# Napoliee/Expressive-FastSpeech2-Mandarin

Measured on AMD Instinct MI355X. Metric: mel-frames/sec/GPU (batch-64 synth) at 1/2/4/8 MI355X; RTF, higher is better.
Workload: dtype bf16; 1 GPU; cfg2: batch=64 x 64 phonemes per GPU, ESD-Chinese-Singing-MFA model.yaml, FastSpeech2.forward eval bf16; global_batch=64, seq_len=64, mel_frames_per_gpu_batch=24883, T_max=430, parallelism=dp1 (independent shards, no collective), hip_graph=True

## Files before the change

expressive-fastspeech2-mandarin_amd/csrc/ffn.hip:

```cpp
#include <cstdlib>
#include <type_traits>
#include <utility>

#include "conv_common.h"
#include "fs2_common.h"

namespace {

#ifndef FFN_TRACE
#define FFN_TRACE 0
#endif
#ifndef FFN_ABLATE
#define FFN_ABLATE 0
#endif

constexpr int kD = 256;
constexpr int kChunk = 256;
constexpr int kUnit = 4096;
constexpr int kDepth = 4;

struct FfnArgs {
  ConvArgs e;
  const bf16 *w;
  const float *b1;
// ... 946 lines not shown
      if (hf == 0) {
#pragma unroll
        for (int i = 0; i < N; ++i) xp[i * 64] = pv[i];
      }
      __builtin_amdgcn_s_waitcnt(kLgkm0);
      __builtin_amdgcn_sched_barrier(0);
      __builtin_amdgcn_s_barrier();
      __builtin_amdgcn_sched_barrier(0);
      if (hf == 1) {
#pragma unroll
        for (int i = 0; i < N; ++i) pv[i] = (xp[i * 64] + sv[0][i]) + sv[1][i];
      }
    }
  };
  const rsrc_t wr = make_rsrc(p.w, p.w_bytes);
  auto tile_dma_range = [&](const void *src, uint32_t bytes, int64_t stride, int off, int i0, int i1) {
    const rsrc_t sr = make_rsrc(src, bytes);
    const uint32_t srow = (uint32_t)stride * 2u;
#pragma unroll
    for (int i = i0; i < i1; ++i) {
      const int pc = wv + NW * i;
      const int o = pc * 1024 + lane * 16;
      const int r = o / XPITCH, within = o - r * XPITCH;
      const int gm = m0 - pad + r;
      const bool ok = r < XROWS && within < 512 && gm >= 0 && gm < M;
      __builtin_amdgcn_raw_ptr_buffer_load_lds(
          sr, (__attribute__((address_space(3))) void *)(smem + off + pc * 1024), 16,
          ok ? (uint32_t)gm * srow + (uint32_t)within : kOOB, 0, 0, 0);
    }
  };
  constexpr uint32_t W2_BASE = (uint32_t)(F * KS * kD * 2);
  const uint32_t lane_off = (uint32_t)lane * 16u + (uint32_t)hf * 2048u;
  auto base1 = [&](int c) { return (uint32_t)((c * 4 + w) * NK1) * (uint32_t)kUnit; };
  auto base2 = [&](int c) { return W2_BASE + (uint32_t)(w * (F / 32) + c * NK2) * (uint32_t)kUnit; };
  bf16x8 pa[DEPTH][JB];
  auto load_at = [&](auto S, uint32_t so) {
    constexpr int s = decltype(S)::value;
    if (FFN_ABLATE & 2) return;
    __builtin_amdgcn_sched_barrier(0);
#pragma unroll
    for (int jb = 0; jb < JB; ++jb) {
      auto v = __builtin_amdgcn_raw_buffer_load_b128(wr, lane_off + jb * 1024, (FFN_ABLATE & 8) ? 0u : so, 0);
      pa[s][jb] = __builtin_bit_cast(bf16x8, v);
    }
    __builtin_amdgcn_sched_barrier(0);
  };
  auto ring_start = [&]() {
    static_for<DEPTH>([&](auto I) { load_at(I, base1(c0) + (uint32_t)(decltype(I)::value * kUnit)); });
  };
  {
    const int hr = lane & 15, hq = lane >> 4;
    if (wv < 3) vec_dma(wv == 0 ? p.bfc : wv == 1 ? p.g1 : p.be1, 0, smem + VEC0_OFF + wv * 1024);
    const rsrc_t fr = make_rsrc(p.wfc, (uint32_t)(kD * kD * 2));
    const uint32_t lane_o = lane_off;
    bf16x8 wf[8][JB];
#pragma unroll
    for (int ks = 0; ks < 8; ++ks)
#pragma unroll
      for (int jb = 0; jb < JB; ++jb)
        wf[ks][jb] = __builtin_bit_cast(bf16x8, __builtin_amdgcn_raw_buffer_load_b128(
                                                    fr, lane_o + (uint32_t)(jb * 1024), (uint32_t)((w * 8 + ks) * kUnit), 0));
    constexpr int PRE_SPLIT = (64 * XPITCH + 1023) / 1024 / NW + 1;
    static_assert(NW * PRE_SPLIT * 1024 >= 64 * XPITCH && PRE_SPLIT <= XP_PER_WAVE, "row pass 0 pieces");
    tile_dma_range(p.att, p.att_bytes, p.as, ATT_OFF, 0, PRE_SPLIT);
    tile_dma_range(a.x, a.x_bytes, a.xs, X_OFF, 0, PRE_SPLIT);
    tile_dma_range(p.att, p.att_bytes, p.as, ATT_OFF, PRE_SPLIT, XP_PER_WAVE);
    tile_dma_range(a.x, a.x_bytes, a.xs, X_OFF, PRE_SPLIT, XP_PER_WAVE);
    stamp(21);
    __builtin_amdgcn_s_waitcnt(vm_imm(2 * (XP_PER_WAVE - PRE_SPLIT)));
    __builtin_amdgcn_s_waitcnt(kLgkm0);
    __builtin_amdgcn_s_barrier();
    stamp(22);
    float *red0 = reinterpret_cast<float *>(smem + RED0_OFF);
    static_for<(XROWS + 63) / 64>([&](auto PS) {
      constexpr int ps = decltype(PS)::value;
      if constexpr (ps == 1) {
        asm volatile("s_waitcnt vmcnt(0)" ::: "memory");
        __builtin_amdgcn_s_barrier();
      }
      f32x4 a0[JB][4];
#pragma unroll
      for (int jb = 0; jb < JB; ++jb)
#pragma unroll
        for (int mb = 0; mb < 4; ++mb) a0[jb][mb] = f32x4{0.f, 0.f, 0.f, 0.f};
#pragma unroll
      for (int ks = 0; ks < 8; ++ks) {
        bf16x8 fb[4];
#pragma unroll
        for (int mb = 0; mb < 4; ++mb) {
          const int r = min(64 * ps + 16 * mb + hr, XROWS - 1);
          fb[mb] = *reinterpret_cast<const bf16x8 *>(smem + ATT_OFF + r * XPITCH + ks * 64 + hq * 16);
        }
#pragma unroll
        for (int mb = 0; mb < 4; ++mb)
#pragma unroll
          for (int jb = 0; jb < JB; ++jb)
            a0[jb][mb] = __builtin_amdgcn_mfma_f32_16x16x32_bf16(wf[ks][jb], fb[mb], a0[jb][mb], 0, 0, 0);
      }
      float part[4] = {0.f, 0.f, 0.f, 0.f}, mean[4], var[4];
      float sv[JB][4];
#pragma unroll
      for (int jb = 0; jb < JB; ++jb) {
        const int n = col0 + jb * 16 + 4 * hq;
        const float4 bb = *reinterpret_cast<const float4 *>(smem + VEC0_OFF + 4 * n);
#pragma unroll
        for (int mb = 0; mb < 4; ++mb) {
          const int r = 64 * ps + 16 * mb + hr, gm = m0 - pad + r;
          const bool ok = r < XROWS && gm >= 0 && gm < M;
          bf16x4 xv = {(bf16)0.f, (bf16)0.f, (bf16)0.f, (bf16)0.f};
          if (ok) xv = *reinterpret_cast<const bf16x4 *>(smem + X_OFF + r * XPITCH + n * 2);
          f32x4 v = a0[jb][mb];
          v[0] = v[0] + bb.x + (float)xv[0];
          v[1] = v[1] + bb.y + (float)xv[1];
          v[2] = v[2] + bb.z + (float)xv[2];
          v[3] = v[3] + bb.w + (float)xv[3];
          a0[jb][mb] = v;
          if constexpr (NW == 8) {
            sv[jb][mb] = (v[0] + v[1]) + (v[2] + v[3]);
            part[mb] += sv[jb][mb];
          } else {
            part[mb] += (v[0] + v[1]) + (v[2] + v[3]);
          }
        }
      }
      auto reduce4 = [&](float (&pv)[4], float (&tot)[4]) {
        pair_sum(pv, sv);
        float t[4];
#pragma unroll
        for (int mb = 0; mb < 4; ++mb) t[mb] = __shfl_xor(pv[mb], 16, 64);
#pragma unroll
        for (int mb = 0; mb < 4; ++mb) pv[mb] += t[mb];
#pragma unroll
        for (int mb = 0; mb < 4; ++mb) t[mb] = __shfl_xor(pv[mb], 32, 64);
        if (NW == 4 || hf == 1) {
#pragma unroll
          for (int mb = 0; mb < 4; ++mb) red0[(mb * 16 + hr) * 4 + w] = pv[mb] + t[mb];
        }
        __builtin_amdgcn_s_waitcnt(kLgkm0);
        __builtin_amdgcn_s_barrier();
#pragma unroll
        for (int mb = 0; mb < 4; ++mb) {
          const float4 r4 = *reinterpret_cast<const float4 *>(red0 + (mb * 16 + hr) * 4);
          tot[mb] = (r4.x + r4.y) + (r4.z + r4.w);
        }
        __builtin_amdgcn_s_waitcnt(kLgkm0);
        __builtin_amdgcn_s_barrier();
      };
      reduce4(part, mean);
#pragma unroll
      for (int mb = 0; mb < 4; ++mb) {
        mean[mb] *= 1.0f / kD;
        float ss = 0.f;
#pragma unroll
        for (int jb = 0; jb < JB; ++jb) {
          f32x4 d = a0[jb][mb];
          d[0] -= mean[mb];
          d[1] -= mean[mb];
          d[2] -= mean[mb];
          d[3] -= mean[mb];
          a0[jb][mb] = d;
          if constexpr (NW == 8) {
            if constexpr (ps == 0)
              sv[jb][mb] = sumsq4<true>(d);
            else if (jb == 0 && mb < 3 && hf == 0)
              sv[jb][mb] = sumsq4<true>(d);
            else
              sv[jb][mb] = sumsq4<false>(d);
            ss += sv[jb][mb];
          } else {
            ss += (d[0] * d[0] + d[1] * d[1]) + (d[2] * d[2] + d[3] * d[3]);
          }
        }
        part[mb] = ss;
      }
      reduce4(part, var);
      float rstd[4], keep[4] = {1.f, 1.f, 1.f, 1.f};
#pragma unroll
      for (int mb = 0; mb < 4; ++mb) rstd[mb] = 1.0f / sqrtf(var[mb] * (1.0f / kD) + p.eps1);
      if (NW == 4 && a.lens != nullptr) {
#pragma unroll
        for (int mb = 0; mb < 4; ++mb) {
          const int gm = m0 - pad + 64 * ps + 16 * mb + hr;
          if (gm >= 0 && gm < M) {
            const int bb = gm / T;
            keep[mb] = (int64_t)(gm - bb * T) < a.lens[bb] ? 1.0f : 0.0f;
          }
        }
      }
#pragma unroll
      for (int jb = 0; jb < JB; ++jb) {
        const int n = col0 + jb * 16 + 4 * hq;
        const float4 g = *reinterpret_cast<const float4 *>(smem + VEC0_OFF + 4 * (kD + n));
        const float4 be = *reinterpret_cast<const float4 *>(smem + VEC0_OFF + 4 * (2 * kD + n));
#pragma unroll
        for (int mb = 0; mb < 4; ++mb) {
          const int r = 64 * ps + 16 * mb + hr;
          const f32x4 d = a0[jb][mb];
          bf16x4 o;
          o[0] = (bf16)((d[0] * rstd[mb] * g.x + be.x) * keep[mb]);
          o[1] = (bf16)((d[1] * rstd[mb] * g.y + be.y) * keep[mb]);
          o[2] = (bf16)((d[2] * rstd[mb] * g.z + be.z) * keep[mb]);
          o[3] = (bf16)((d[3] * rstd[mb] * g.w + be.w) * keep[mb]);
          if (r < XROWS) *reinterpret_cast<bf16x4 *>(smem + X_OFF + r * XPITCH + n * 2) = o;
        }
      }
      stamp(23 + ps);
    });
    __builtin_amdgcn_s_waitcnt(kLgkm0);
    __builtin_amdgcn_s_barrier();
    load_vectors();
    ring_start();
  }


  const int hrow0 = lane & 15;
  const int hi = lane >> 4;
  bf16x8 f0[MB], f1[MB];
  auto bases_x = [&](int tap, int (&ad)[MB]) {
    const int base = X_OFF + (hrow0 + tap) * XPITCH + hi * 16;
#pragma unroll
    for (int mb = 0; mb < MB; ++mb) {
      const int keep = (FFN_ABLATE & 16) ? -1 : __builtin_amdgcn_sbfe(vmask[mb], tap, 1);
      ad[mb] = (base + mb * 16 * XPITCH) & keep;
    }
  };
  auto issue_x = [&](const int (&ad)[MB], auto KSI, bf16x8 (&f)[MB]) {
    if (FFN_ABLATE & 4) return;
    constexpr int off = decltype(KSI)::value * 64;
#pragma unroll
    for (int mb = 0; mb < MB; ++mb) f[mb] = *reinterpret_cast<const bf16x8 *>(smem + ad[mb] + off);
  };
  auto read_h = [&](int q, bf16x8 (&f)[MB]) {
    if (FFN_ABLATE & 4) return;
    const char *hp = smem + H_OFF + hrow0 * 512 + (xchunk(hrow0, 4 * q + hi) << 4);
#pragma unroll
    for (int mb = 0; mb < MB; ++mb) f[mb] = *reinterpret_cast<const bf16x8 *>(hp + mb * 8192);
  };

  f32x4 acc1[JB][MB], acc2[JB][MB];
#pragma unroll
  for (int i = 0; i < JB; ++i)
#pragma unroll
    for (int j = 0; j < MB; ++j) {
      acc1[i][j] = f32x4{0.f, 0.f, 0.f, 0.f};
      acc2[i][j] = f32x4{0.f, 0.f, 0.f, 0.f};
    }
  auto mma = [&](f32x4 (&acc)[JB][MB], const bf16x8 (&fa)[JB], const bf16x8 (&fb)[MB]) {
    if (FFN_ABLATE & 1) return;
#pragma unroll
    for (int mb = 0; mb < MB; ++mb)
#pragma unroll
      for (int jb = 0; jb < JB; ++jb)
        acc[jb][mb] = __builtin_amdgcn_mfma_f32_16x16x32_bf16(fa[jb], fb[mb], acc[jb][mb], 0, 0, 0);
  };
  auto bar = []() {
    __builtin_amdgcn_sched_barrier(0);
    __builtin_amdgcn_s_barrier();
    __builtin_amdgcn_sched_barrier(0);
  };
  auto trace_dump = [&](int last) {
    if (FFN_TRACE) {
      uint64_t *o = S > 1 ? reinterpret_cast<uint64_t *>(static_cast<char *>(p.part) + p.part_bytes + 256u * blockIdx.x)
                          : reinterpret_cast<uint64_t *>(static_cast<char *>(a.out) + (size_t)(a.M - 1 - blockIdx.x) * a.os * 2);
      for (int i = 0; i < 25; ++i) o[i] = *reinterpret_cast<const uint64_t *>(smem + SMEM + 8 * i);
      o[28] = t_entry;
      o[29] = (uint64_t)split;
      o[30] = (uint64_t)last;
      o[31] = (uint64_t)25;
    }
  };
  stamp(0);

  auto write_h = [&](int c) {
    float z;
    asm volatile("v_mov_b32 %0, 0" : "=v"(z));
#pragma unroll
    for (int jb = 0; jb < JB; ++jb) {
      const int j = col0 + jb * 16 + 4 * hi;
      const float4 bb = *reinterpret_cast<const float4 *>(smem + B1_OFF + 4 * (c * kChunk + j));
#pragma unroll
      for (int mb = 0; mb < MB; ++mb) {
        const f32x4 v = acc1[jb][mb];
        bf16x4 o;
        o[0] = (bf16)fmaxf(v[0] + bb.x, 0.f);
        o[1] = (bf16)fmaxf(v[1] + bb.y, 0.f);
        o[2] = (bf16)fmaxf(v[2] + bb.z, 0.f);
        o[3] = (bf16)fmaxf(v[3] + bb.w, 0.f);
        const int m = hrow0 + mb * 16;
        *reinterpret_cast<bf16x4 *>(smem + H_OFF + m * 512 + (xchunk(m, j >> 3) << 4) + (j & 7) * 2) = o;
        acc1[jb][mb] = f32x4{z, z, z, z};
      }
    }
  };

  asm volatile("s_waitcnt vmcnt(%0)" ::"n"(JB * DEPTH) : "memory");
  __builtin_amdgcn_s_waitcnt(kLgkm0);
  bar();
  stamp(1);
  int bxc[MB], bxn[MB];
  bases_x(0, bxc);
  issue_x(bxc, std::integral_constant<int, 0>{}, f0);

  static_assert(DEPTH == 4 && kD / 32 == 8, "8 units per tap, 4-unit ring");
  auto unit1 = [&](auto KSI, int c, int tap) {
    constexpr int ks = decltype(KSI)::value, s = ks % DEPTH;
    if constexpr (ks + 1 < 8) {
      if constexpr (ks & 1)
        issue_x(bxc, std::integral_constant<int, ks + 1>{}, f0);
      else
        issue_x(bxc, std::integral_constant<int, ks + 1>{}, f1);
    } else {
      issue_x(bxn, std::integral_constant<int, 0>{}, f0);
    }
    if constexpr (ks & 1)
      mma(acc1, pa[s], f1);
    else
      mma(acc1, pa[s], f0);
    const uint32_t k1 = (uint32_t)(tap * 8 + ks + DEPTH) * (uint32_t)kUnit;
    if constexpr (ks + DEPTH < 8) {
      load_at(std::integral_constant<int, s>{}, base1(c) + k1);
    } else {
      const bool more = tap + 1 < KS;
      load_at(std::integral_constant<int, s>{},
              more ? base1(c) + k1 : base2(c) + (uint32_t)(((2 * w + ks - DEPTH) & (NK2 - 1)) * kUnit));
    }
  };
#pragma nounroll
  for (int c = c0; c < cend; ++c) {
#pragma nounroll
    for (int tap = 0; tap < KS; ++tap) {
      bases_x(tap + 1, bxn);
      static_for<8>([&](auto KSI) { unit1(KSI, c, tap); });
#pragma unroll
      for (int mb = 0; mb < MB; ++mb) bxc[mb] = bxn[mb];
    }
    stamp(2 + 2 * (c - c0));
    bar();
    write_h(c);
    __builtin_amdgcn_s_waitcnt(kLgkm0);
    stamp(3 + 2 * (c - c0));
    if constexpr (NW == 8) bar();
    read_h(2 * w, f0);
    const uint32_t next1 = c + 1 < cend ? base1(c + 1) : 0u;
    static_for<NK2>([&](auto Q) {
      constexpr int q = decltype(Q)::value;
      constexpr int s = q % DEPTH;
      if constexpr (q == 1 && NW == 4) {
        __builtin_amdgcn_s_waitcnt(kLgkm0);
        bar();
      }
      const int qn = (2 * w + q + 1) & (NK2 - 1);
      if constexpr (q + 1 == NK2) {
        bases_x(0, bxc);
        issue_x(bxc, std::integral_constant<int, 0>{}, f0);
      }
      else if constexpr (q & 1)
        read_h(qn, f0);
      else
        read_h(qn, f1);
      if constexpr (q & 1)
        mma(acc2, pa[s], f1);
      else
        mma(acc2, pa[s], f0);
      if constexpr (q + DEPTH < NK2)
        load_at(std::integral_constant<int, s>{}, base2(c) + (uint32_t)(((2 * w + q + DEPTH) & (NK2 - 1)) * kUnit));
      else
        load_at(std::integral_constant<int, s>{}, next1 + (uint32_t)((q + DEPTH - NK2) * kUnit));
    });
  }

  stamp(2 + 2 * NCH);
  asm volatile("s_waitcnt vmcnt(0)" ::: "memory");
  __builtin_amdgcn_s_waitcnt(kLgkm0);
  stamp(4 + 2 * NCH);
  {
    int lane_e = lane;
    if constexpr (NW == 8) asm volatile("" : "+v"(lane_e));
    const int hrow0 = lane_e & 15, hi = lane_e >> 4;
    float *red = reinterpret_cast<float *>(smem + RED_OFF);
    const float inv_n = 1.0f / 256.0f;
    float4 b2v[JB], gv[JB], bev[JB];
#pragma unroll
    for (int nb = 0; nb < JB; ++nb) {
      const int n = col0 + nb * 16 + 4 * hi;
      b2v[nb] = *reinterpret_cast<const float4 *>(smem + EP_OFF + 4 * n);
      gv[nb] = *reinterpret_cast<const float4 *>(smem + EP_OFF + 4 * (kD + n));
      bev[nb] = *reinterpret_cast<const float4 *>(smem + EP_OFF + 4 * (2 * kD + n));
    }
    float part[MB];
    float sv[JB][MB];
#pragma unroll
    for (int mb = 0; mb < MB; ++mb) {
      const int xr = mb * 16 + hrow0 + pad;
      float sum = 0.f;
#pragma unroll
      for (int nb = 0; nb < JB; ++nb) {
        const int n = col0 + nb * 16 + 4 * hi;
        const bf16x4 xv = *reinterpret_cast<const bf16x4 *>(smem + X_OFF + xr * XPITCH + n * 2);
        f32x4 v = acc2[nb][mb];
        v[0] = v[0] + b2v[nb].x + (float)xv[0];
        v[1] = v[1] + b2v[nb].y + (float)xv[1];
        v[2] = v[2] + b2v[nb].z + (float)xv[2];
        v[3] = v[3] + b2v[nb].w + (float)xv[3];
        acc2[nb][mb] = v;
        if constexpr (NW == 8) {
          sv[nb][mb] = (v[0] + v[1]) + (v[2] + v[3]);
          sum += sv[nb][mb];
        } else {
          sum += (v[0] + v[1]) + (v[2] + v[3]);
        }
      }
      part[mb] = sum;
    }
    auto row_reduce = [&](float (&pv)[MB], float (&tot)[MB]) {
      pair_sum(pv, sv);
      float t[MB];
#pragma unroll
      for (int mb = 0; mb < MB; ++mb) t[mb] = __shfl_xor(pv[mb], 16, 64);
#pragma unroll
      for (int mb = 0; mb < MB; ++mb) pv[mb] += t[mb];
#pragma unroll
      for (int mb = 0; mb < MB; ++mb) t[mb] = __shfl_xor(pv[mb], 32, 64);
      if (NW == 4 || hf == 1) {
#pragma unroll
        for (int mb = 0; mb < MB; ++mb) red[(mb * 16 + hrow0) * 4 + w] = pv[mb] + t[mb];
      }
      __syncthreads();
#pragma unroll
      for (int mb = 0; mb < MB; ++mb) {
        const float4 r = *reinterpret_cast<const float4 *>(red + (mb * 16 + hrow0) * 4);
        tot[mb] = (r.x + r.y) + (r.z + r.w);
      }
      __syncthreads();
    };
    float mean[MB], var[MB];
    stamp(14);
    row_reduce(part, mean);
    stamp(15);
#pragma unroll
    for (int mb = 0; mb < MB; ++mb) {
      mean[mb] *= inv_n;
      float ss = 0.f;
#pragma unroll
      for (int nb = 0; nb < JB; ++nb) {
        f32x4 d = acc2[nb][mb];
        d[0] -= mean[mb];
        d[1] -= mean[mb];
        d[2] -= mean[mb];
        d[3] -= mean[mb];
        acc2[nb][mb] = d;
        if constexpr (NW == 8) {
          sv[nb][mb] = sumsq4<false>(d);
          ss += sv[nb][mb];
        } else {
          ss += (d[0] * d[0] + d[1] * d[1]) + (d[2] * d[2] + d[3] * d[3]);
        }
      }
      part[mb] = ss;
    }
    stamp(16);
    row_reduce(part, var);
    stamp(17);
    auto finish = [&](auto PADDED) {
      constexpr bool padded = decltype(PADDED)::value;
#pragma unroll
      for (int mb = 0; mb < MB; ++mb) {
        const float rstd = 1.0f / sqrtf(var[mb] * inv_n + a.eps);
        const int m = mb * 16 + hrow0;
        bool masked = false;
        int bb = 0;
        if constexpr (padded) {
          bb = (m0 + m) / T;
          masked = (padmask >> mb) & 1;
        }
#pragma unroll
        for (int nb = 0; nb < JB; ++nb) {
          const int n = col0 + nb * 16 + 4 * hi;
          const f32x4 d = acc2[nb][mb];
          float y[4] = {d[0] * rstd * gv[nb].x + bev[nb].x, d[1] * rstd * gv[nb].y + bev[nb].y,
                        d[2] * rstd * gv[nb].z + bev[nb].z, d[3] * rstd * gv[nb].w + bev[nb].w};
          if constexpr (padded) {
            if (masked) y[0] = y[1] = y[2] = y[3] = 0.f;
            if (a.av1 != nullptr) {
              const float4 v1 = *reinterpret_cast<const float4 *>(a.av1 + (int64_t)bb * kD + n);
              y[0] += v1.x; y[1] += v1.y; y[2] += v1.z; y[3] += v1.w;
            }
            if (a.av2 != nullptr) {
              const float4 v2 = *reinterpret_cast<const float4 *>(a.av2 + (int64_t)bb * kD + n);
              y[0] += v2.x; y[1] += v2.y; y[2] += v2.z; y[3] += v2.w;
            }
          }
          bf16x4 o;
          o[0] = (bf16)y[0];
          o[1] = (bf16)y[1];
          o[2] = (bf16)y[2];
          o[3] = (bf16)y[3];
          *reinterpret_cast<bf16x4 *>(smem + H_OFF + m * 512 + (xchunk(m, n >> 3) << 4) + (n & 7) * 2) = o;
        }
      }
    };
    if (NW == 4 && (a.lens != nullptr || a.av1 != nullptr || a.av2 != nullptr))
      finish(std::true_type{});
    else
      finish(std::false_type{});
    __syncthreads();
    stamp(18);
    const uint32_t orow = (uint32_t)a.os * 2u;
    char *ob = static_cast<char *>(a.out);
#pragma unroll 2
    for (int i = tid; i < BM * 32; i += NT) {
      const int m = i >> 5, ch = i & 31;
      if (m0 + m < M) {
        const uint4 v = *reinterpret_cast<const uint4 *>(smem + H_OFF + m * 512 + (xchunk(m, ch) << 4));
        if (p.out_sc1)
          __builtin_amdgcn_raw_buffer_store_b128(__builtin_bit_cast(__attribute__((ext_vector_type(4))) unsigned, v),
                                                 make_rsrc(ob, 0x7fffffffu), (uint32_t)((m0 + m) * orow + ch * 16), 0, 16);
        else
          *reinterpret_cast<uint4 *>(ob + (size_t)(m0 + m) * orow + ch * 16) = v;
      }
    }
    if (p.wq != nullptr) {
      const rsrc_t qr = make_rsrc(p.wq, p.wq_bytes);
      auto qload = [&](auto S, uint32_t so) {
        constexpr int s = decltype(S)::value;
        __builtin_amdgcn_sched_barrier(0);
#pragma unroll
        for (int jb = 0; jb < JB; ++jb) {
          auto v = __builtin_amdgcn_raw_buffer_load_b128(qr, lane_off + jb * 1024, so, 0);
          pa[s][jb] = __builtin_bit_cast(bf16x8, v);
        }
        __builtin_amdgcn_sched_barrier(0);
      };
      constexpr int SPITCH = 528;
      const uint32_t qrow = (uint32_t)p.qs * 2u;
      char *qb = reinterpret_cast<char *>(p.qkv);
      const int npass = p.nq / 256;
      auto qbase = [&](int ps) { return (uint32_t)((ps * 4 + w) * 8) * (uint32_t)kUnit; };
      auto lbar = [&]() {
        __builtin_amdgcn_s_waitcnt(kLgkm0);
        __builtin_amdgcn_sched_barrier(0);
        __builtin_amdgcn_s_barrier();
        __builtin_amdgcn_sched_barrier(0);
      };
      static_for<DEPTH>([&](auto I) { qload(I, qbase(0) + (uint32_t)(decltype(I)::value * kUnit)); });
#pragma nounroll
      for (int ps = 0; ps < npass; ++ps) {
        const uint32_t base = qbase(ps);
        float z;
        asm volatile("v_mov_b32 %0, 0" : "=v"(z));
#pragma unroll
        for (int jb = 0; jb < JB; ++jb)
#pragma unroll
          for (int mb = 0; mb < MB; ++mb) acc1[jb][mb] = f32x4{z, z, z, z};
        read_h(0, f0);
        static_for<8>([&](auto Q) {
          constexpr int q = decltype(Q)::value, sl = q % DEPTH;
          if constexpr (q + 1 < 8) {
            if constexpr (q & 1)
              read_h(q + 1, f0);
            else
              read_h(q + 1, f1);
          }
          if constexpr (q & 1)
            mma(acc1, pa[sl], f1);
          else
            mma(acc1, pa[sl], f0);
          if constexpr (q + DEPTH < 8)
            qload(std::integral_constant<int, sl>{}, base + (uint32_t)((q + DEPTH) * kUnit));
          else
            qload(std::integral_constant<int, sl>{},
                  (ps + 1 < npass ? qbase(ps + 1) : qbase(0)) + (uint32_t)((q + DEPTH - 8) * kUnit));
        });
#pragma unroll
        for (int jb = 0; jb < JB; ++jb) {
          const int c = col0 + jb * 16 + 4 * hi;
          const float4 bb = *reinterpret_cast<const float4 *>(p.bq + ps * 256 + c);
#pragma unroll
          for (int mb = 0; mb < MB; ++mb) {
            const f32x4 v = acc1[jb][mb];
            bf16x4 o;
            o[0] = (bf16)(v[0] + bb.x);
            o[1] = (bf16)(v[1] + bb.y);
            o[2] = (bf16)(v[2] + bb.z);
            o[3] = (bf16)(v[3] + bb.w);
            *reinterpret_cast<bf16x4 *>(smem + X_OFF + (hrow0 + mb * 16) * SPITCH + c * 2) = o;
          }
        }
        lbar();
#pragma unroll 2
        for (int i = tid; i < BM * 32; i += NT) {
          const int m = i >> 5, ch = i & 31;
          if (m0 + m < M) {
            const uint4 v = *reinterpret_cast<const uint4 *>(smem + X_OFF + m * SPITCH + ch * 16);
            if (p.out_sc1)
              __builtin_amdgcn_raw_buffer_store_b128(__builtin_bit_cast(__attribute__((ext_vector_type(4))) unsigned, v),
                                                     make_rsrc(qb, 0x7fffffffu),
                                                     (uint32_t)((m0 + m) * qrow + ps * 512 + ch * 16), 0, 16);
            else
              *reinterpret_cast<uint4 *>(qb + (size_t)(m0 + m) * qrow + ps * 512 + ch * 16) = v;
          }
        }
        lbar();
      }
      asm volatile("s_waitcnt vmcnt(0)" ::: "memory");
    }
  }
  stamp(5 + 2 * NCH);
  if (FFN_TRACE) {
    stamp(3 + 2 * NCH);
    __syncthreads();
    if (tid == 0) trace_dump(1);
  }
}

}

extern "C" int fs2_ffn(const fs2_ffn_desc *d, fs2_stream_t stream) {
  if (d == nullptr || d->x == nullptr || d->w == nullptr || d->b1 == nullptr || d->b2 == nullptr ||
      d->ln_gamma == nullptr || d->ln_beta == nullptr || d->out == nullptr)
    return FS2_EINVAL;
  if (d->B < 0 || d->T < 0 || d->x_row_stride < kD || (d->x_row_stride & 7) || d->out_row_stride < kD ||
      (d->out_row_stride & 7))
    return FS2_EINVAL;
  if (d->D != kD || !(d->F == 1024 || d->F == 512) || !(d->KS == 9 || d->KS == 3) || d->pad < 0 ||
      d->pad > d->KS - 1)
    return FS2_EUNSUPPORTED;
  if ((d->rows_dev == nullptr) != (d->row_pos == nullptr)) return FS2_EINVAL;
  if (d->rows_dev != nullptr && (d->lens != nullptr || d->addvec1 != nullptr || d->addvec2 != nullptr))
    return FS2_EINVAL;
  if (d->x == d->out) return FS2_EINVAL;
  const int S = d->nsplit <= 1 ? 1 : d->nsplit;
  if (!(S == 1 || S == 2 || S == 4) || S > d->F / kChunk) return FS2_EINVAL;
  const int64_t M64 = (int64_t)d->B * d->T;
  if (M64 > 0x7fffff00LL) return FS2_EINVAL;
  if (M64 == 0) return FS2_OK;
  const int64_t xb = M64 * d->x_row_stride * 2;
  const int64_t wb = ffn_weight_elems(d->KS, d->F) * 2;
  if (xb >= (1LL << 31)) return FS2_EUNSUPPORTED;

  FfnArgs p{};
  ConvArgs &a = p.e;
  a = ConvArgs{};
  a.x = d->x;
  a.xs = d->x_row_stride;
  a.w = d->w;
  a.bias = d->b2;
  a.B = d->B;
  a.T = d->T;
  a.Cin = kD;
  a.Cin_pad = kD;
  a.N = kD;
  a.KS = d->KS;
  a.pad = d->pad;
  a.M = (int)M64;
  a.epi = FS2_EPI_RES_LN;
  a.res = d->x;
  a.res_dt = FS2_BF16;
  a.rs = d->x_row_stride;
  a.gamma = d->ln_gamma;
  a.beta = d->ln_beta;
  a.eps = d->ln_eps;
  a.lens = d->lens;
  a.av1 = d->addvec1;
  a.av2 = d->addvec2;
  a.out = d->out;
  a.out_dt = FS2_BF16;
  a.os = d->out_row_stride;
  a.rows_dev = d->rows_dev;
  a.row_pos = reinterpret_cast<const int2 *>(d->row_pos);
  a.out_scale = 1.0f;
  a.ln_pairs = 1;
#ifdef FFN_EPI_DBG
  a.dbg = FFN_EPI_DBG;
#endif
  a.x_bytes = (uint32_t)xb;
  a.w_bytes = (uint32_t)wb;
  p.w = reinterpret_cast<const bf16 *>(d->w);
  p.b1 = d->b1;
  p.w_bytes = (uint32_t)wb;
// ... 112 lines not shown
```

Baseline: 18.48 million mel-frames/s.

## Software-pipeline FFN conv taps across chunks to hide the H-buffer barrier

Restructures the FFN conv-tap loop so the first tap of the next chunk runs between write_h and the barrier that guards the H buffer, and the barrier moves after tap 1. Weight-load addresses are now passed as precomputed current/next bases with a wrap offset, instead of being recomputed from chunk and tap indices with selects. The aim is to overlap MFMA work with the LDS write/barrier stall and to drop two extra barriers, including the NW==4 barrier inside the second GEMM. The lane index in the epilogue is recomputed through mbcnt, presumably to ease register pressure. The more complex address and wrap logic adds some risk of correctness or scheduling regressions.

```diff
diff --git a/expressive-fastspeech2-mandarin_amd/csrc/ffn.hip b/expressive-fastspeech2-mandarin_amd/csrc/ffn.hip
--- a/expressive-fastspeech2-mandarin_amd/csrc/ffn.hip
+++ b/expressive-fastspeech2-mandarin_amd/csrc/ffn.hip
@@ -1272,7 +1272,7 @@
   issue_x(bxc, std::integral_constant<int, 0>{}, f0);
 
   static_assert(DEPTH == 4 && kD / 32 == 8, "8 units per tap, 4-unit ring");
-  auto unit1 = [&](auto KSI, int c, int tap) {
+  auto unit1 = [&](auto KSI, uint32_t cur, uint32_t nxt, int wrap) {
     constexpr int ks = decltype(KSI)::value, s = ks % DEPTH;
     if constexpr (ks + 1 < 8) {
       if constexpr (ks & 1)
@@ -1286,42 +1286,52 @@
       mma(acc1, pa[s], f1);
     else
       mma(acc1, pa[s], f0);
-    const uint32_t k1 = (uint32_t)(tap * 8 + ks + DEPTH) * (uint32_t)kUnit;
-    if constexpr (ks + DEPTH < 8) {
-      load_at(std::integral_constant<int, s>{}, base1(c) + k1);
-    } else {
-      const bool more = tap + 1 < KS;
+    if constexpr (ks + DEPTH < 8)
+      load_at(std::integral_constant<int, s>{}, cur + (uint32_t)((ks + DEPTH) * kUnit));
+    else
       load_at(std::integral_constant<int, s>{},
-              more ? base1(c) + k1 : base2(c) + (uint32_t)(((2 * w + ks - DEPTH) & (NK2 - 1)) * kUnit));
-    }
-  };
+              nxt + (uint32_t)((ks + DEPTH - 8) * kUnit) - (ks + DEPTH - 8 >= wrap ? (uint32_t)(NK2 * kUnit) : 0u));
+  };
+  auto tap1 = [&](int tapn, uint32_t cur, uint32_t nxt, int wrap = 4) {
+    bases_x(tapn, bxn);
+    static_for<8>([&](auto KSI) { unit1(KSI, cur, nxt, wrap); });
+#pragma unroll
+    for (int mb = 0; mb < MB; ++mb) bxc[mb] = bxn[mb];
+  };
+  static_assert(KS >= 3, "tap 0 ahead, tap 1 ahead of the guard, a last tap after it");
+  constexpr uint32_t kTap = 8u * (uint32_t)kUnit;
+  auto opaque = [](int v) {
+    asm volatile("" : "+s"(v));
+    return v;
+  };
+  tap1(1, base1(c0), base1(c0) + kTap);
 #pragma nounroll
   for (int c = c0; c < cend; ++c) {
+    const bool lastc = c + 1 == cend;
+    const uint32_t cb = base1(c), nb = lastc ? 0u : base1(c + 1);
+    const uint32_t g2 = base2(c) + (uint32_t)(2 * w * kUnit);
+    const int g2wrap = NK2 - 2 * w;
+    tap1(opaque(2), cb + kTap, cb + 2u * kTap);
+    bar();
 #pragma nounroll
-    for (int tap = 0; tap < KS; ++tap) {
-      bases_x(tap + 1, bxn);
-      static_for<8>([&](auto KSI) { unit1(KSI, c, tap); });
-#pragma unroll
-      for (int mb = 0; mb < MB; ++mb) bxc[mb] = bxn[mb];
+    for (int tap = 2; tap < KS; ++tap) {
+      const bool lastt = tap + 1 == KS;
+      tap1(lastt ? 0 : tap + 1, cb + (uint32_t)tap * kTap, lastt ? (lastc ? g2 : nb) : cb + (uint32_t)(tap + 1) * kTap,
+           lastt && lastc ? g2wrap : 4);
     }
     stamp(2 + 2 * (c - c0));
-    bar();
     write_h(c);
     __builtin_amdgcn_s_waitcnt(kLgkm0);
     stamp(3 + 2 * (c - c0));
-    if constexpr (NW == 8) bar();
+    if (!lastc) tap1(opaque(1), nb, g2, g2wrap);
+    bar();
     read_h(2 * w, f0);
-    const uint32_t next1 = c + 1 < cend ? base1(c + 1) : 0u;
+    const uint32_t next1 = nb + (lastc ? 0u : kTap);
     static_for<NK2>([&](auto Q) {
       constexpr int q = decltype(Q)::value;
       constexpr int s = q % DEPTH;
-      if constexpr (q == 1 && NW == 4) {
-        __builtin_amdgcn_s_waitcnt(kLgkm0);
-        bar();
-      }
       const int qn = (2 * w + q + 1) & (NK2 - 1);
       if constexpr (q + 1 == NK2) {
-        bases_x(0, bxc);
         issue_x(bxc, std::integral_constant<int, 0>{}, f0);
       }
       else if constexpr (q & 1)
@@ -1344,7 +1354,7 @@
   __builtin_amdgcn_s_waitcnt(kLgkm0);
   stamp(4 + 2 * NCH);
   {
-    int lane_e = lane;
+    int lane_e = (int)__builtin_amdgcn_mbcnt_hi(~0u, __builtin_amdgcn_mbcnt_lo(~0u, 0u));
     if constexpr (NW == 8) asm volatile("" : "+v"(lane_e));
     const int hrow0 = lane_e & 15, hi = lane_e >> 4;
     float *red = reinterpret_cast<float *>(smem + RED_OFF);
```

After: 18.56 million mel-frames/s, median of 6. About the same (+0.4%).
